# aslpavel/svgrasterize.py

Measured on AMD Instinct MI355X. Metric: Mpixels/sec AA coverage+composite (path-pixels/s; whole step: flatten+binning+coverage+composite; planned replay -- a frame with new geometry: value_replan), higher is better.
Workload: dtype f64 arithmetic, f32 RGBA store; 1 GPU; synthetic 4096 random closed cubic paths @ 4096x4096 (SURVEY 8d generator, splitmix64 0x5F3759DF); edges=783607

## Files before the change

### svgrasterize.py_amd/csrc/svgr_hip.hip

```cpp
#include <hip/hip_runtime.h>

#include <algorithm>
#include <atomic>
#include <cstdarg>
#include <cstddef>
#include <cmath>
#include <cstdio>
#include <cstring>
#include <ctime>
#include <initializer_list>
#include <new>
#include <string>
#include <type_traits>
#include <vector>
#include <memory>
#include <unordered_map>
#include <utility>

#include "../../include/svgr.h"
#include "svgr_core.h"

using namespace svgr;

static std::atomic<unsigned long long> g_n_launches{0};
// ... 719 lines not shown
        if (i0 + PER <= n) {
            ((int4*)(seg_off + i0))[0] = make_int4(o[0], o[1], o[2], o[3]);
            ((int4*)(seg_off + i0))[1] = make_int4(o[4], o[5], o[6], o[7]);
        } else {
#pragma unroll
            for (int k = 0; k < PER; ++k)
                if (i0 + k < n) seg_off[i0 + k] = o[k];
        }
        __syncthreads();
        if (tid == 0) s_run = run0 + all;
        __syncthreads();
    }
    if (tid == 0) seg_off[n] = s_run;
}

struct PathBin {
    int b0, nb;
    int pb_off;
    int cell_off;
};
__host__ __device__ __forceinline__ void path_ctiles(int c0, int cols, int vc0, int& ct0, int& nct) {
    span_ctiles(c0, cols, vc0, TC, ct0, nct);
}
static_assert(sizeof(PathBin) == 16, "PathBin is one dwordx4");

constexpr int PB_THREADS = 256;
constexpr int PB_CELLS = 80;
constexpr int PB_BANDS = 16;
static_assert(PB_BANDS * TR <= PB_THREADS && PB_BANDS <= PB_CELLS, "k_path_build: one lane group per band of the slab");
struct Slab {
    int p, band0, nb, k0;
    int nk, e_begin, e_end, pb_off;
    int r0, c0, rows, cols;
    int b0, cell_off, pad[2];
};
static_assert(sizeof(Slab) == 64, "Slab is four dwordx4");
__host__ __device__ __forceinline__ void slab_shape(int nb, int nct, int& bands_per, int& col_runs) {
    if (nct <= PB_CELLS) {
        bands_per = PB_CELLS / nct < PB_BANDS ? PB_CELLS / nct : PB_BANDS;
        col_runs = 1;
    } else {
        bands_per = 1;
        col_runs = (nct + PB_CELLS - 1) / PB_CELLS;
    }
    (void)nb;
}

__global__ __launch_bounds__(64) void k_path_bbox(const unsigned long long* __restrict__ pkeys, int n_paths, int has_vp,
                                                  int vr0, int vc0, int vrows, int vcols, int* __restrict__ bbox,
                                                  PathBin* __restrict__ bins, BatchDev* __restrict__ bd, int stats,
                                                  const int* __restrict__ plist, Slab* __restrict__ slabs, int slab_cap, Owner own,
                                                  const int* __restrict__ path_seg0, const int* __restrict__ seg_off, int edge_cap,
                                                  const int* __restrict__ slab_at) {
    const int pi = blockIdx.x * blockDim.x + threadIdx.x, lane = threadIdx.x & 63;
    const int p = plist ? (pi < n_paths ? plist[pi] : 0x7fffffff) : pi;
    if (plist) n_paths = pi < n_paths ? 0x7fffffff : 0;
    int e_begin = 0, e_end = 0;
    if (slabs && p < n_paths) {
        e_begin = seg_off[path_seg0[p]]; e_end = seg_off[path_seg0[p + 1]];
    }
    const bool reuse = slab_at != nullptr;
    PathBin old_bin;
    old_bin.b0 = old_bin.nb = old_bin.pb_off = old_bin.cell_off = 0;
    int4 old_bb = make_int4(0, 0, 0, 0);
    if (reuse && p < n_paths) { old_bin = bins[p]; old_bb = ((const int4*)bbox)[p]; }
    int out[4] = {0, 0, 0, 0};
    int pb0 = 0, pnb = 0, pnct = 0;
    int st_n = 0;
    unsigned long long st_px = 0;
    unsigned st_minr = 0, st_minc = 0, st_maxr = 0, st_maxc = 0;
    PathBox pb = path_box(0ull, 0ull, 0ull, 0ull, has_vp, vr0, vc0, vrows, vcols, TR, TC);
    if (p < n_paths) {
        const unsigned long long* k = pkeys + 4 * (size_t)p;
        pb = path_box(k[0], k[1], k[2], k[3], has_vp, vr0, vc0, vrows, vcols, TR, TC);
        if (pb.refused) atomicOr(&bd->err, 16);
        out[0] = pb.r0; out[1] = pb.c0; out[2] = pb.rows; out[3] = pb.cols;
        pb0 = pb.b0; pnb = pb.nb; pnct = pb.nct;
        if (pb.rows > 0 && pb.cols > 0) {
            st_n = 1;
            st_px = (unsigned long long)((long long)pb.rows * pb.cols);
            st_minr = (unsigned)(UNION_BIAS - pb.r0);
            st_minc = (unsigned)(UNION_BIAS - pb.c0);
            st_maxr = (unsigned)(UNION_BIAS + (pb.r0 + pb.rows));
            st_maxc = (unsigned)(UNION_BIAS + (pb.c0 + pb.cols));
        }
    }
    if (reuse && p < n_paths && !path_box_is(pb, old_bb.x, old_bb.y, old_bb.z, old_bb.w, old_bin.nb)) {
        atomicOr(&bd->err, 32);
        out[0] = old_bb.x; out[1] = old_bb.y; out[2] = old_bb.z; out[3] = old_bb.w;
        pb0 = old_bin.b0; pnb = old_bin.nb; pnct = 0;
        if (pnb > 0 && out[2] > 0 && out[3] > 0) {
            int ct0_;
// ... 42 lines not shown
        st_n += __shfl_xor(st_n, d);
        st_px += __shfl_xor(st_px, d);
        unsigned a = __shfl_xor(st_minr, d), b = __shfl_xor(st_minc, d), c = __shfl_xor(st_maxr, d), e = __shfl_xor(st_maxc, d);
        st_minr = a > st_minr ? a : st_minr; st_minc = b > st_minc ? b : st_minc;
        st_maxr = c > st_maxr ? c : st_maxr; st_maxc = e > st_maxc ? e : st_maxc;
    }
    if (stats && lane == 0 && st_n > 0) {
        atomicAdd(&bd->n_nonempty, st_n);
        atomicAdd(&bd->path_pixels, st_px);
        atomicMax(&bd->umin_r, st_minr);
        atomicMax(&bd->umin_c, st_minc);
        atomicMax(&bd->umax_r, st_maxr);
        atomicMax(&bd->umax_c, st_maxc);
    }
    const bool coop = slabs != nullptr && own.world <= 1;
    if (coop) {
        const bool fits = n_slabs > 0 && slab0 + n_slabs <= slab_cap;
        int t_sl;
        const int e_sl = wave_excl_scan(fits ? n_slabs : 0, lane, t_sl);
        const int eb = e_begin < edge_cap ? e_begin : edge_cap, ee = e_end < edge_cap ? e_end : edge_cap;
        for (int base = 0; base < t_sl; base += 64) {
            const int i = base + lane;
            int owner = 0;
#pragma unroll
            for (int step = 32; step >= 1; step >>= 1) {
                const int cand = owner + step;
                const int first = __shfl(e_sl, cand & 63);
                if (cand < 64 && first <= i) owner = cand;
            }
            const int o_first = __shfl(e_sl, owner), o_slab0 = __shfl(slab0, owner), o_p = __shfl(p, owner);
            const int o_pb0 = __shfl(pb0, owner), o_pnb = __shfl(pnb, owner), o_pnct = __shfl(pnct, owner);
            const int o_bper = __shfl(bands_per, owner), o_cruns = __shfl(col_runs, owner);
            const int o_eb = __shfl(eb, owner), o_ee = __shfl(ee, owner), o_off = __shfl(off, owner), o_cell = __shfl(cell_off, owner);
            const int o_r0 = __shfl(out[0], owner), o_c0 = __shfl(out[1], owner), o_rows = __shfl(out[2], owner), o_cols = __shfl(out[3], owner);
            if (i < t_sl) {
                const int j = i - o_first;
                const int br = o_cruns == 1 ? j : j / o_cruns, c = o_cruns == 1 ? 0 : j - br * o_cruns;
                const int bb = br * o_bper, be = bb + o_bper < o_pnb ? bb + o_bper : o_pnb;
                Slab sl;
                sl.p = o_p; sl.band0 = o_pb0 + bb; sl.nb = be - bb;
                sl.k0 = c * PB_CELLS; sl.nk = o_pnct - sl.k0 < PB_CELLS ? o_pnct - sl.k0 : PB_CELLS;
                sl.e_begin = o_eb; sl.e_end = o_ee; sl.pb_off = o_off;
                sl.r0 = o_r0; sl.c0 = o_c0; sl.rows = o_rows; sl.cols = o_cols;
                sl.b0 = o_pb0; sl.cell_off = o_cell;
                sl.pad[0] = sl.pad[1] = 0;
                slabs[o_slab0 + j] = sl;
            }
        }
    }
    if (slabs && n_slabs > 0 && !(coop && slab0 + n_slabs <= slab_cap)) {
        if (slab0 + n_slabs > slab_cap) {
            atomicOr(&bd->err, 4);
            for (int at = slab0; at < slab_cap; ++at) {
                Slab sl;
                memset(&sl, 0, sizeof sl);
                slabs[at] = sl;
            }
        } else {
            int at = slab0;
            e_begin = e_begin < edge_cap ? e_begin : edge_cap;
            e_end = e_end < edge_cap ? e_end : edge_cap;
            for (int bb = 0; bb < pnb; bb += bands_per) {
                const int be = bb + bands_per < pnb ? bb + bands_per : pnb;
                if (!owns_any(own, pb0 + bb, pb0 + be - 1)) continue;
                for (int c = 0; c < col_runs; ++c) {
                    Slab sl;
                    sl.p = p; sl.band0 = pb0 + bb; sl.nb = be - bb;
                    sl.k0 = c * PB_CELLS; sl.nk = pnct - sl.k0 < PB_CELLS ? pnct - sl.k0 : PB_CELLS;
                    sl.e_begin = e_begin; sl.e_end = e_end; sl.pb_off = off;
                    sl.r0 = out[0]; sl.c0 = out[1]; sl.rows = out[2]; sl.cols = out[3];
                    sl.b0 = pb0; sl.cell_off = cell_off;
                    sl.pad[0] = sl.pad[1] = 0;
                    slabs[at++] = sl;
                }
            }
        }
    }
    if (p < n_paths) {
        ((int4*)bbox)[p] = make_int4(out[0], out[1], out[2], out[3]);
        PathBin pbin;
        pbin.b0 = pb0; pbin.nb = pnb; pbin.pb_off = off; pbin.cell_off = cell_off;
        bins[p] = pbin;
    }
}

__device__ __forceinline__ bool edge_prepare(const double* __restrict__ edges, const int* __restrict__ edge_path,
                                             const int* __restrict__ bbox, int e, EdgeSetup& es, int& p, int& r0) {
    p = edge_path[e];
    const int4 bb = ((const int4*)bbox)[p];
    r0 = bb.x;
    const int rows = bb.z, cols = bb.w;
    if (rows <= 0 || cols <= 0) return false;
    const double o_r = (double)bb.x, o_c = (double)bb.y;
    const double* ed = edges + 4 * (size_t)e;
    double ar = ed[0] - o_r, ac = ed[1] - o_c, br = ed[2] - o_r, bc = ed[3] - o_c;
    es = edge_setup(ar, ac, br, bc, rows);
    if (!es.valid) return false;
    double cmin = ac < bc ? ac : bc;
    if (cmin >= (double)cols + 2.0) return false;
    return true;
}

__device__ __forceinline__ void band_rows(const EdgeSetup& es, int band, int vr0, int r0, int& ya, int& yb) {
    const int b0row = band * TR + vr0 - r0;
    ya = es.y_begin > b0row ? es.y_begin : b0row;
// ... 186 lines not shown

__device__ __forceinline__ int lds_col(int tcol) {
    static_assert((PX & (PX - 1)) == 0, "PX is a power of two");
    return tcol + (int)((unsigned)tcol / PX) * (CHUNK_STRIDE - PX);
}
__device__ __forceinline__ int lds_index(int trow, int tcol) {
    return __mul24(trow, ROW_STRIDE) + lds_col(tcol);
}
__device__ __forceinline__ int run_pieces(int tcol, int len) {
    return ((tcol + len - 1) / PX) - (tcol / PX) + 1;
}
__device__ __forceinline__ unsigned add_where(int trow, int tcol, int len) {
    return (unsigned)(lds_index(trow, tcol) * 8) | ((unsigned)(len - 1) << 16) | ((unsigned)(tcol & (PX - 1)) << 22);
}

struct EdgeLds {
    double p0y, p1y, dxdy, x;
};
__device__ __forceinline__ double replay_rows(double x, int y, int n, double p0y, double p1y, double dxdy) {
    if (n <= 0) return x;
    RowState st;
    st.x_next = x; st.x = x; st.d = 0.0;
    row_step(st, y, p0y, p1y, dxdy, 1.0);
    double xn = st.x_next;
    for (int k = 1; k < n; ++k) xn = xn + dxdy;
    return xn;
}
static_assert(sizeof(EdgeLds) == 32, "EdgeLds is two 16-byte LDS reads (its first row and direction ride in an int array beside it)");
constexpr int PB_BATCH = 256;
constexpr int PB_EPL = (PB_BATCH + PB_THREADS - 1) / PB_THREADS;
static_assert(PB_BATCH % 64 == 0 && PB_BATCH / 16 <= 32, "two-level search: at most 32 coarse entries, read four at a time");
static_assert(PB_BANDS * TR * PB_BATCH < (1 << 20) && PB_BATCH < (1 << 11), "stage() scans row counts and live flags in one packed word");
constexpr int PB_WAVES = 6;
__device__ __forceinline__ void pb_barrier() { asm volatile("s_waitcnt lgkmcnt(0)\n\ts_barrier" ::: "memory"); }
template <int MODE>
__global__ __launch_bounds__(PB_THREADS, PB_WAVES) void k_path_build(const Slab* __restrict__ slabs, const double* __restrict__ edges,
                                                           const int* __restrict__ pair_idx, const double* __restrict__ path_paint,
                                                           const uint8_t* __restrict__ path_rule, const int* __restrict__ path_group,
                                                           const int* __restrict__ path_grad, int vr0, int vc0, int n_ct, int mask_words,
                                                           unsigned long long* __restrict__ tile_mask, CellHdr* __restrict__ cell_hdr,
                                                           int cell_cap, const AddShards ash, TileAdd* __restrict__ adds,
                                                           int2* __restrict__ cell_plan, BatchDev* __restrict__ bd, Owner own, int stats, int det,
                                                           unsigned long long* __restrict__ dbg,
                                                           const unsigned long long* __restrict__ guard_keys, const int* __restrict__ guard_bbox,
                                                           const PathBin* __restrict__ guard_bins, int n_paths, int vrows, int vcols) {
#ifdef SVGR_DBG_PB_STAMP
#define PB_STAMP(i) do { if (threadIdx.x == 0 && dbg && blockIdx.x < 8192) dbg[8 * blockIdx.x + (i)] = __builtin_amdgcn_s_memrealtime(); } while (0)
#else
#define PB_STAMP(i) do { } while (0)
#endif
    constexpr bool PLANNED = MODE != 0;
    constexpr bool BOUNDED = MODE == 2;
    PB_STAMP(0);
    __shared__ __attribute__((aligned(16))) double s_sum[PB_CELLS * TR];
    __shared__ double s_left[TR];
    __shared__ int s_cnt[PB_CELLS], s_pos[PB_CELLS], s_plan_n[PB_CELLS];
    __shared__ unsigned s_rowb[PB_CELLS + 1];
    __shared__ __attribute__((aligned(16))) EdgeLds s_edge[PB_BATCH];
    __shared__ int s_eya[PB_BATCH];
    __shared__ __attribute__((aligned(16))) int s_pref[PB_BATCH + 4];
    __shared__ unsigned short s_start[PB_THREADS];
    __shared__ int s_wtot[PB_EPL][PB_THREADS / 64];
    __shared__ __attribute__((aligned(8))) int2 s_info[PB_CELLS];
    __shared__ unsigned s_rowm[PB_CELLS];
    __shared__ int s_ptot[PB_BANDS], s_pidx[PB_BANDS], s_base, s_ok;
    const int tid = threadIdx.x, lane = tid & 63, wave = tid >> 6;
    for (int i = tid; i < PB_CELLS * TR / 2; i += PB_THREADS) ((double2*)s_sum)[i] = make_double2(0.0, 0.0);
    for (int i = tid; i < PB_CELLS; i += PB_THREADS) {
        s_cnt[i] = 0; s_pos[i] = (int)0x80000000; s_plan_n[i] = 0; s_rowb[i] = 0u; s_info[i] = make_int2(0, 0);
    }
    if (tid < TR) s_left[tid] = 0.0;
    if (tid == 0) s_rowb[PB_CELLS] = 0u;
    const Slab sl = slabs[blockIdx.x];
    const bool guarding = MODE == 1 && guard_keys != nullptr;
    const int n_slabs_now = guarding ? (int)gridDim.x : bd->slab_cursor;
    if ((int)blockIdx.x >= n_slabs_now) return;
    if (sl.nb <= 0 || sl.nk <= 0) return;
    PB_STAMP(7);
    const int p = sl.p;
    const int r0 = sl.r0, c0 = sl.c0, rows = sl.rows, cols = sl.cols;
    int ct0, nct;
    path_ctiles(c0, cols, vc0, ct0, nct);
    const int x_first = vc0 + ct0 * TC - c0;
    const int e_begin = sl.e_begin, e_end = sl.e_end;
    const int sr0 = vr0 + sl.band0 * TR - r0, sr1 = sr0 + sl.nb * TR;
    const int n_cell = sl.nb * sl.nk;
    const double o_r = (double)r0, o_c = (double)c0;
    const int rl = path_rule[p], rule = rl & 1;
    const int group = path_group ? path_group[p] : -1;
    const int grad1 = path_grad ? path_grad[p] + 1 : 0;
    const double4 paint = ((const double4*)path_paint)[p];
    auto cell_of = [&](int g, int k) { return sl.cell_off + (sl.band0 + g - sl.b0) * nct + sl.k0 + k; };
    int s_per = 0;
    int2 my_plan = make_int2((int)0x80000000, 0);
    bool plan_pending = false;
    int my_pidx = 0;
    if ((tid & (TR - 1)) == 0 && tid / TR < sl.nb && owns_band(own, sl.band0 + tid / TR)) my_pidx = pair_idx[sl.pb_off + sl.band0 + tid / TR - sl.b0];
    if (PLANNED && !BOUNDED) {
        if (tid < n_cell) {
            const int g = tid / sl.nk, k = tid - g * sl.nk;
            const int cell = cell_of(g, k);
            if (cell < cell_cap) my_plan = cell_plan[cell];
        }
        plan_pending = true;
    }

    auto stage = [&](int eb, bool bounds = false) -> int {
        int cnt[PB_EPL], eya[PB_EPL];
        EdgeLds el[PB_EPL];
#pragma unroll
        for (int j = 0; j < PB_EPL; ++j) {
            const int e = eb + tid + j * PB_THREADS;
            cnt[j] = 0;
            el[j].p0y = el[j].p1y = el[j].dxdy = el[j].x = 0.0; eya[j] = 0;
            if (e < e_end && tid + j * PB_THREADS < PB_BATCH) {
                const double4 ed = ((const double4*)edges)[e];
                const double ar = ed.x - o_r, ac = ed.y - o_c, br = ed.z - o_r, bc = ed.w - o_c;
                const EdgeSetup es = edge_setup(ar, ac, br, bc, rows);
                const double cmin = ac < bc ? ac : bc;
                if (es.valid && !(cmin >= (double)cols + 2.0)) {
                    const int ya = es.y_begin > sr0 ? es.y_begin : sr0, yb = es.y_end < sr1 ? es.y_end : sr1;
                    if (ya < yb) {
                        cnt[j] = yb - ya;
                        el[j].p0y = es.p0y; el[j].p1y = es.p1y; el[j].dxdy = es.dxdy; el[j].x = replay_rows(es.x, es.y_begin, ya - es.y_begin, es.p0y, es.p1y, es.dxdy);
                        eya[j] = ya | (es.dir < 0.0 ? (int)0x80000000 : 0);
                    }
                }
            }
        }
#ifdef SVGR_DBG_PB_STAMP
        if (PLANNED && eb == e_begin) { asm volatile("s_waitcnt vmcnt(0)" ::: "memory"); PB_STAMP(5); }
#endif
        int excl[PB_EPL], wtot[PB_EPL];
#pragma unroll
        for (int j = 0; j < PB_EPL; ++j) excl[j] = wave_excl_scan(cnt[j] | ((cnt[j] > 0 ? 1 : 0) << 20), lane, wtot[j]);
        pb_barrier();
        if (PLANNED && plan_pending) {
            if (tid < PB_CELLS) { s_pos[tid] = my_plan.x; s_plan_n[tid] = my_plan.y; }
            plan_pending = false;
        }
        if (BOUNDED && bounds) {
#pragma unroll
            for (int j = 0; j < PB_EPL; ++j) {
                if (cnt[j] <= 0) continue;
                const int ya = eya[j] & 0x7fffffff, yb = ya + cnt[j];
                const double dx = el[j].dxdy;
                const double ylo = (double)ya > el[j].p0y ? (double)ya : el[j].p0y;
                for (int y0 = ya; y0 < yb;) {
                    const int vrow = r0 + y0 - vr0, band = vrow / TR;
// ... 154 lines not shown
            if (ne == 0) continue;
            const int ci = bl * sl.nk + (k - sl.k0);
            const int pos = __hip_atomic_fetch_add(&s_cnt[ci], ne, __ATOMIC_RELAXED, __HIP_MEMORY_SCOPE_WORKGROUP);
            __hip_atomic_fetch_add(&s_sum[ci * TR + trow], part, __ATOMIC_RELAXED, __HIP_MEMORY_SCOPE_WORKGROUP);
            __hip_atomic_fetch_or(&s_rowb[ci], 1u << trow, __ATOMIC_RELAXED, __HIP_MEMORY_SCOPE_WORKGROUP);
            if (STORE) {
                const int first = s_pos[ci];
                if (first < 0 || pos + ne > s_plan_n[ci]) continue;
                store_pieces(ra, trow, ca, cb, cell_c0, adds + ((size_t)first + pos));
            }
        }
    };
    auto emit_row = [&](const RowAt& ra) {
        if (!((ra.where >> 16) & 1)) return;
        const int bl = ra.where & 0xff, trow = (ra.where >> 8) & 0xff;
        int kf, kl;
        row_tiles(ra, kf, kl);
        kf = kf > sl.k0 ? kf : sl.k0;
        for (int k = kf; k <= kl; ++k) {
            int ca, cb;
            tile_cols(k, ca, cb);
            int ne = 0;
            const int cell_c0 = k * TC + x_first;
            record_adds(ra.x0i, ra.n, ra.v, ca, cb, [&](int, double) { ++ne; },
                        [&](int c, int len, double) { ne += run_pieces(c - cell_c0, len); });
            if (ne == 0) continue;
            const int ci = bl * sl.nk + (k - sl.k0);
            const int pos = __hip_atomic_fetch_add(&s_pos[ci], ne, __ATOMIC_RELAXED, __HIP_MEMORY_SCOPE_WORKGROUP);
            if (pos < 0) continue;
            store_pieces(ra, trow, ca, cb, cell_c0, adds + pos);
        }
    };

    const bool one_batch = e_end - e_begin <= PB_BATCH;
    int total = 0, n_rows = 0;
    if (BOUNDED) {
        for (int eb = e_begin; eb < e_end; eb += PB_BATCH) {
            total = stage(eb, true);
            n_rows += total;
        }
        PB_STAMP(1);
        static_assert(PB_CELLS <= 128, "the cells' places: a prefix sum by the first two waves");
        int room = 0, excl = 0;
        if (tid < 128) {
            const int bnd = tid < n_cell ? s_plan_n[tid] : 0;
            const int gg = tid < n_cell ? tid / sl.nk : 0, kk = tid < n_cell ? tid - gg * sl.nk : 0;
            const bool ends_here = cols - ((sl.k0 + kk) * TC + x_first) < TC;
            const int b_lo = vr0 + (sl.band0 + gg) * TR - r0;
            const int rin = (b_lo + TR < rows ? b_lo + TR : rows) - (b_lo > 0 ? b_lo : 0);
            room = bnd > 0 ? bnd + rin + (ends_here ? rin : 0) : 0;
            int wt;
            excl = wave_excl_scan(room, lane, wt);
            if (lane == 0) s_ptot[wave] = wt;
        }
        pb_barrier();
        if (tid == 0) {
            const int all = s_ptot[0] + s_ptot[1];
            const int sh = p % ash.n;
            int at = 0;
            if (all > 0) at = atomicAdd(&bd->shard[sh].add_cursor, all);
            int ok = 1;
            if ((long long)at + all > (long long)ash.cap[sh]) { atomicOr(&bd->err, 64); ok = 0; }
            s_base = ash.base[sh] + at;
            s_ok = ok;
        }
        pb_barrier();
        if (tid < n_cell) s_pos[tid] = room > 0 && s_ok ? s_base + (wave ? s_ptot[0] : 0) + excl : (int)0x80000000;
        pb_barrier();
        if (one_batch) {
            for_rows(total, [&](const RowAt& ra) { count_row(ra, std::true_type{}); });
        } else {
            for (int eb = e_begin; eb < e_end; eb += PB_BATCH) {
                const int tot = stage(eb);
                for_rows(tot, [&](const RowAt& ra) { count_row(ra, std::true_type{}); });
            }
        }
    } else
    for (int eb = e_begin; eb < e_end; eb += PB_BATCH) {
        total = stage(eb);
        PB_STAMP(1);
        n_rows += total;
        if (PLANNED) for_rows(total, [&](const RowAt& ra) { count_row(ra, std::true_type{}); });
        else for_rows(total, [&](const RowAt& ra) { count_row(ra, std::false_type{}); });
    }
    if (stats && tid == 0 && n_rows > 0) atomicAdd(&bd->bseg_cursor, n_rows);
    if (guarding && __builtin_amdgcn_readfirstlane(wave) == 0) {
        const int grid = (int)gridDim.x, g0 = ((int)blockIdx.x + grid - grid / 2) % grid;
        for (int g = g0; g * 64 < n_paths; g += grid) {
            const int q = g * 64 + lane;
            if (q >= n_paths) continue;
            const unsigned long long* k = guard_keys + 4 * (size_t)q;
            const int4 bb = ((const int4*)guard_bbox)[q];
            const PathBox pb = path_box(k[0], k[1], k[2], k[3], 1, vr0, vc0, vrows, vcols, TR, TC);
            if (pb.refused) atomicOr(&bd->err, 16);
            if (!path_box_is(pb, bb.x, bb.y, bb.z, bb.w, guard_bins[q].nb)) atomicOr(&bd->err, 32);
        }
    }
    pb_barrier();
    PB_STAMP(2);
    auto write_cell = [&](int g, int k, int cls, double cin, unsigned cm, unsigned sm, int own_n, int n_list, int add0, int row_l, int idx,
                          bool slab_ok) -> bool {
        const int band = sl.band0 + g;
        const int cell = cell_of(g, k);
        const bool mask_ok = (unsigned)(idx >> 6) < (unsigned)mask_words;
        if (!(cell < cell_cap && slab_ok && mask_ok) || (PLANNED && cls == 2 && add0 < 0)) {
            if (row_l == 0) atomicOr(&bd->err, 32);
            return false;
        }
        CellHdr* hd = cell_hdr + cell;
        if (cls == 1) hd->carry[row_l] = cin;
        const int cell_c0 = (sl.k0 + k) * TC + x_first;
        const unsigned below = (1u << row_l) - 1u;
        const int n_carry = __popc(cm);
        if (((cm >> row_l) & 1u) && adds) {
            store_add(adds + ((size_t)add0 + own_n + __popc(cm & below)), add_where(row_l, cell_c0 < 0 ? -cell_c0 : 0, 1), cin);
        }
        if (((sm >> row_l) & 1u) && adds) {
            store_add(adds + ((size_t)add0 + own_n + n_carry + __popc(sm & below)), add_where(row_l, cols - cell_c0, 1), __builtin_nan(""));
        }
        if (row_l == 0) {
            unsigned long long* const mw = tile_mask + ((size_t)band * n_ct + ct0 + sl.k0 + k) * 2 * mask_words + (idx >> 6);
            const unsigned long long mbit = 1ull << (idx & 63);
            atomicOr(mw, mbit);
            if (cls == 2) atomicOr(mw + mask_words, mbit);
            hd->paint[0] = paint.x; hd->paint[1] = paint.y; hd->paint[2] = paint.z; hd->paint[3] = paint.w;
            hd->r0 = r0; hd->c0 = c0; hd->rows = rows; hd->cols = cols;
            hd->bits = rule | (((rl >> 1) & 3) << 1) | (cls << 3) | (grad1 << 5);
            hd->n_add = n_list; hd->add0 = add0; hd->p = p;
            hd->group = group;
        }
        return true;
    };
// ... 2438 lines not shown
        SVGR_LAUNCH(k_path_rows, grid1((size_t)ns), dim3(256), 0, st, (const double*)b->segs.p, (const uint8_t*)b->seg_kind.p,
                           (const int*)b->seg_path.p, (const double*)b->path_m6.p, ns, b->prow());
        prow = b->prow();
    }
    const int n_bands_vp = use_vp ? (b->vp[2] + TR - 1) / TR : 0;
    if (upto <= 1) {
        if (upto == 1) {
            if (int rc = b->seg_cnt.ensure((size_t)ns + 1)) return rc;
            if (int rc = b->seg_off.ensure((size_t)ns + 2)) return rc;
            if (int rc = b->lane_off.ensure(((size_t)ns << fl_sub) + 1)) return rc;
            if (listed || prow) HIPCHK(hipMemsetAsync(b->seg_cnt.p, 0, sizeof(int) * ((size_t)ns + 1), st));
        }
        if (ns > 0) {
            auto launch_cnt = [&](auto kern) {
                SVGR_LAUNCH(kern, fgrid, dim3(FL_BLOCK), 0, st, (const double*)b->segs.p,
                                   (const uint8_t*)b->seg_kind.p, (const int*)b->seg_path.p, (const double*)b->path_m6.p, ns,
                                   b->thr, (double*)nullptr, (int*)nullptr, b->shards, b->pkeys(), b->bd(), b->own, b->vp[0],
                                   n_bands_vp, prow, seg_list, n_items, upto == 1 ? b->seg_cnt.p : (int*)nullptr, (const int*)nullptr,
                                   use_vp ? b->vp[3] : 0 ,
                                   upto == 1 ? b->lane_off.p : (int*)nullptr, (int*)nullptr, (unsigned long long*)nullptr);
            };
            if (fl_sub == 6) launch_cnt(k_flatten<false, false, 6>); else launch_cnt(k_flatten<false, false, 5>);
        }
        if (upto == 1 && !b->late_scan)
            SVGR_LAUNCH(k_seg_scan, dim3(1), dim3(1024), 0, st, (const int*)b->seg_cnt.p, ns, b->seg_off.p);
        if (upto == 0 || (upto == 1 && b->census_bbox)) {
            b->slabs_current = false;
            SVGR_LAUNCH(k_path_bbox, grid1((size_t)std::max(np_walk, 1), 64), dim3(64), 0, st, (const unsigned long long*)b->pkeys(),
                               np_walk, use_vp ? 1 : 0, b->vp[0], b->vp[1], b->vp[2], b->vp[3], b->bbox.p, b->bins.p, b->bd(), 1, plist,
                               (Slab*)nullptr, 0, b->own, (const int*)nullptr, (const int*)nullptr, 0, (const int*)nullptr);
        }
        return 0;
    }
    if (ns > 0) {
        const bool lane_places = !b->safe_path;
        auto launch_fl = [&](auto kern, int* places) {
            SVGR_LAUNCH(kern, fgrid, dim3(FL_BLOCK), 0, st, (const double*)b->segs.p,
                               (const uint8_t*)b->seg_kind.p, (const int*)b->seg_path.p, (const double*)b->path_m6.p, ns, b->thr,
                               b->edges.p, b->edge_path.p, b->shards, b->pkeys(), b->bd(), b->own, b->vp[0],
                               n_bands_vp, prow, seg_list, n_items, (int*)nullptr, (const int*)b->seg_off.p,
                               cap_i32(std::min(b->edge_path.cap, b->edges.cap / 4)), places, (int*)nullptr, (unsigned long long*)nullptr);
        };
        const bool placed_fl = lane_places && b->lane_off.p && b->lane_off.cap >= ((size_t)ns << fl_sub);
        if (b->fl_scan) {
            auto launch_scan = [&](auto kern) {
                SVGR_LAUNCH(kern, fgrid, dim3(FL_BLOCK), 0, st, (const double*)b->segs.p,
                                   (const uint8_t*)b->seg_kind.p, (const int*)b->seg_path.p, (const double*)b->path_m6.p, ns, b->thr,
                                   b->edges.p, b->edge_path.p, b->shards, b->pkeys(), b->bd(), b->own, b->vp[0],
                                   n_bands_vp, prow, seg_list, n_items, b->seg_cnt.p, (const int*)nullptr,
                                   cap_i32(std::min(b->edge_path.cap, b->edges.cap / 4)), b->lane_off.p, b->seg_off.p, b->scan_state());
            };
            if (fl_sub == 6) launch_scan(k_flatten<true, false, 6, true>); else launch_scan(k_flatten<true, false, 5, true>);
        } else if (fl_sub == 6) {
            if (placed_fl) launch_fl(k_flatten<true, true, 6>, b->lane_off.p); else launch_fl(k_flatten<true, false, 6>, (int*)nullptr);
        } else {
            if (placed_fl) launch_fl(k_flatten<true, true, 5>, b->lane_off.p); else launch_fl(k_flatten<true, false, 5>, (int*)nullptr);
        }
    }
    const bool keep_lists = upto >= 4 && b->planned && b->slab_at_valid && use_vp && !b->safe_path;
    const bool placed = b->planned && b->add_places && b->slab_at_valid && !b->count_adds_only && b->cell_plan.p != nullptr;
    const svgr_batch::SlabsMade slabs_now{b->slabs.p, b->bbox.p, b->bins.p, b->slab_at.p, b->n_slabs, b->n_paths, {b->vp[0], b->vp[1], b->vp[2], b->vp[3]}};
    const bool slabs_for_plan = keep_lists && b->own.world <= 1 && !listed && ns > 0 && b->n_slabs > 0 && b->n_slabs <= (int64_t)cap_i32(b->slabs.cap);
    const bool keep_slabs = slabs_for_plan && placed && b->slabs_current && b->slabs_made == slabs_now;
    if (!keep_slabs) {
        SVGR_LAUNCH(k_path_bbox, grid1((size_t)std::max(np_walk, 1), 64), dim3(64), 0, st, (const unsigned long long*)b->pkeys(), np_walk,
                           use_vp ? 1 : 0, b->vp[0], b->vp[1], b->vp[2], b->vp[3], b->bbox.p, b->bins.p, b->bd(), b->planned ? 0 : 1, plist,
                           upto >= 3 ? b->slabs.p : (Slab*)nullptr, (int)std::min<int64_t>(cap_i32(b->slabs.cap), b->n_slabs) , b->own,
                           (const int*)b->path_seg0.p, (const int*)b->seg_off.p,
                           cap_i32(std::min(b->edge_path.cap, b->edges.cap / 4)),
                           upto >= 4 && b->planned && b->slab_at_valid ? (const int*)b->slab_at.p : (const int*)nullptr);
        b->slabs_current = slabs_for_plan && !b->slab_order_late;
        b->slab_order_late = false;
        b->slabs_made = slabs_now;
    }
    if (upto == 2) return 0;
    const int owned = count_owned_bands(b->own, b->n_bands);
    const bool clear_in_be = owned > 0 && !keep_lists && upto >= 4 && !b->masks_zeroed && b->tile_mask.p && b->own.world <= 1;
    if (owned > 0 && !keep_lists)
        SVGR_LAUNCH(k_band_entries, dim3(owned), dim3(BE_BLOCK), 0, st, (const PathBin*)b->bins.p, np_walk, plist,
                           (const int*)b->bbox.p, b->band_start.p, b->band_count.p, b->band_item0.p, b->entries.p,
                           b->pair_idx.p, cap_i32(std::min(b->entries.cap, b->pair_idx.cap)),
                           upto >= 4 ? cap_i32(b->items.cap) : 0x7fffffff, b->vp[1], b->bd(), b->own,
                           upto >= 4 && b->planned && use_vp && !b->safe_path ? 1 : 0,
                           clear_in_be ? b->tile_mask.p : (unsigned long long*)nullptr, b->n_ctiles() * 2 * b->mask_words);
    if (clear_in_be) b->masks_zeroed = true;
    if (upto == 3) return 0;
    if (!b->masks_zeroed && b->tile_mask.p) {
        HIPCHK(hipMemsetAsync(b->tile_mask.p, 0, b->mask_bytes(), st));
        b->masks_zeroed = true;
    }
    unsigned long long* pb_dbg = nullptr;
#ifdef SVGR_DBG_PB_STAMP
    {
        static unsigned long long* buf = nullptr;
        if (!buf) { (void)hipMalloc((void**)&buf, 8 * 8 * 8192); (void)hipMemset(buf, 0, 8 * 8 * 8192); }
        pb_dbg = buf;
    }
#endif
    if (b->n_slabs > 0) {
        b->masks_zeroed = false;
        auto launch_pb = [&](auto kern) {
            SVGR_LAUNCH(kern, dim3((unsigned)b->n_slabs), dim3(PB_THREADS), 0, st, (const Slab*)b->slabs.p, (const double*)b->edges.p,
                               (const int*)b->pair_idx.p, (const double*)b->path_paint.p, (const uint8_t*)b->path_rule.p,
                               b->n_groups > 0 ? (const int*)b->path_group.p : (const int*)nullptr,
                               b->n_grads > 0 ? (const int*)b->path_grad.p : (const int*)nullptr, b->vp[0], b->vp[1], b->n_ctiles(), b->mask_words,
                               b->tile_mask.p, b->cell_hdr.p, cap_i32(std::min(b->cell_hdr.cap, b->cell_plan.cap)), b->add_shards,
                               b->count_adds_only ? (TileAdd*)nullptr : b->adds.p, b->cell_plan.p, b->bd(), b->own, b->planned ? 0 : 1,
                               b->deterministic ? 1 : 0, pb_dbg, keep_slabs ? (const unsigned long long*)b->pkeys() : (const unsigned long long*)nullptr,
                               (const int*)b->bbox.p, (const PathBin*)b->bins.p, np, b->vp[2], b->vp[3]);
        };
        const bool bounded = !placed && !b->count_adds_only && b->adds.p && b->adds_roomy && !b->safe_path && !getenv("SVGR_SAFE_PATH");
        if (placed) launch_pb(k_path_build<1>); else if (bounded) launch_pb(k_path_build<2>); else launch_pb(k_path_build<0>);
#ifdef SVGR_DBG_PB_STAMP
        if (pb_dbg && b->planned && !b->count_adds_only) {
            static int n_dump = 0;
            if (++n_dump == 20) {
                HIPCHK(hipStreamSynchronize(st));
                const size_t n = (size_t)std::min<int64_t>(b->n_slabs, 8192);
                std::vector<unsigned long long> h(8 * n);
                HIPCHK(hipMemcpy(h.data(), pb_dbg, sizeof(unsigned long long) * h.size(), hipMemcpyDeviceToHost));
                double ph[5] = {0, 0, 0, 0, 0}, rows_ = 0;
                unsigned long long lo = ~0ull, hi = 0;
                for (size_t i = 0; i < n; ++i) {
                    for (int q = 0; q < 5; ++q) ph[q] += (double)(h[8 * i + q + 1] - h[8 * i + q]);
                    rows_ += (double)h[8 * i + 6];
                    lo = std::min(lo, h[8 * i]); hi = std::max(hi, h[8 * i + 3]);
                }
                double s_rec = 0, s_edges = 0;
                for (size_t i = 0; i < n; ++i) { s_rec += (double)(h[8 * i + 7] - h[8 * i]); s_edges += (double)(h[8 * i + 5] - h[8 * i + 7]); }
                fprintf(stderr, "[pb stamp] %zu slabs, mean us: stage %.2f (slab record %.2f, edges landed +%.2f)  passA %.2f  walk %.2f | rows/slab %.0f | span %.1f us\n", n,
                        ph[0] / n / 100, s_rec / n / 100, s_edges / n / 100, ph[1] / n / 100, ph[2] / n / 100, rows_ / n, (double)(hi - lo) / 100);
                if (const char* f = getenv("SVGR_DBG_PB_DUMP")) { if (FILE* fp = fopen(f, "wb")) { fwrite(h.data(), 8, h.size(), fp); fclose(fp); } }
            }
        }
#endif
    }
    if (owned > 0 && b->n_ctiles() > 0) {
        SVGR_LAUNCH(k_tile_lists, dim3(owned), dim3(TL_BLOCK), 0, st, (const int*)b->band_start.p, (const int*)b->band_item0.p,
                           (const TileEntry*)b->entries.p, b->tile_mask.p, b->mask_words, b->n_ctiles(), b->vp[1], b->own, owned,
                           b->tile_info.p, b->pages.p, b->items.p, (const CellHdr*)b->cell_hdr.p, cap_i32(b->items.cap), cap_i32(b->cell_hdr.cap), b->bd(),
                           keep_lists ? (const PathBin*)b->bins.p : (const PathBin*)nullptr, (const int*)b->bbox.p);
        b->masks_zeroed = true;
    }
    return 0;
}
// ... 2330 lines not shown
```

Before: 810,100 Mpixels/s.

## Fuse planned curve flattening into path-build slabs, skipping the global edge buffer

On planned replay with reusable slabs, the separate flatten kernel is skipped. Each path-build slab re-flattens its path's segments batch by batch straight into shared memory, using the precomputed lane placements, so edges are never written to or read from global memory. The bbox guard check is now folded from keys computed during this flatten, and a small new kernel covers paths that have no slabs. The costs are repeated flattening for paths split across many slabs, an extra barrier per batch, and lower occupancy (5 waves instead of 6).

Measured after the change: 688,900 Mpixels/s. 15.0% lower.

```diff
diff --git a/svgrasterize.py_amd/csrc/svgr_hip.hip b/svgrasterize.py_amd/csrc/svgr_hip.hip
--- a/svgrasterize.py_amd/csrc/svgr_hip.hip
+++ b/svgrasterize.py_amd/csrc/svgr_hip.hip
@@ -775,7 +775,8 @@
     int p, band0, nb, k0;
     int nk, e_begin, e_end, pb_off;
     int r0, c0, rows, cols;
-    int b0, cell_off, pad[2];
+    int b0, cell_off;
+    int seg0, n_seg;
 };
 static_assert(sizeof(Slab) == 64, "Slab is four dwordx4");
 __host__ __device__ __forceinline__ void slab_shape(int nb, int nct, int& bands_per, int& col_runs) {
@@ -798,9 +799,10 @@
     const int pi = blockIdx.x * blockDim.x + threadIdx.x, lane = threadIdx.x & 63;
     const int p = plist ? (pi < n_paths ? plist[pi] : 0x7fffffff) : pi;
     if (plist) n_paths = pi < n_paths ? 0x7fffffff : 0;
-    int e_begin = 0, e_end = 0;
+    int e_begin = 0, e_end = 0, seg_first = 0, seg_n = 0;
     if (slabs && p < n_paths) {
-        e_begin = seg_off[path_seg0[p]]; e_end = seg_off[path_seg0[p + 1]];
+        seg_first = path_seg0[p]; seg_n = path_seg0[p + 1] - seg_first;
+        e_begin = seg_off[seg_first]; e_end = seg_off[seg_first + seg_n];
     }
     const bool reuse = slab_at != nullptr;
     PathBin old_bin;
@@ -909,6 +911,7 @@
             const int o_pb0 = __shfl(pb0, owner), o_pnb = __shfl(pnb, owner), o_pnct = __shfl(pnct, owner);
             const int o_bper = __shfl(bands_per, owner), o_cruns = __shfl(col_runs, owner);
             const int o_eb = __shfl(eb, owner), o_ee = __shfl(ee, owner), o_off = __shfl(off, owner), o_cell = __shfl(cell_off, owner);
+            const int o_seg = __shfl(seg_first, owner), o_nseg = __shfl(seg_n, owner);
             const int o_r0 = __shfl(out[0], owner), o_c0 = __shfl(out[1], owner), o_rows = __shfl(out[2], owner), o_cols = __shfl(out[3], owner);
             if (i < t_sl) {
                 const int j = i - o_first;
@@ -920,7 +923,7 @@
                 sl.e_begin = o_eb; sl.e_end = o_ee; sl.pb_off = o_off;
                 sl.r0 = o_r0; sl.c0 = o_c0; sl.rows = o_rows; sl.cols = o_cols;
                 sl.b0 = o_pb0; sl.cell_off = o_cell;
-                sl.pad[0] = sl.pad[1] = 0;
+                sl.seg0 = o_seg; sl.n_seg = o_nseg;
                 slabs[o_slab0 + j] = sl;
             }
         }
@@ -947,7 +950,7 @@
                     sl.e_begin = e_begin; sl.e_end = e_end; sl.pb_off = off;
                     sl.r0 = out[0]; sl.c0 = out[1]; sl.rows = out[2]; sl.cols = out[3];
                     sl.b0 = pb0; sl.cell_off = cell_off;
-                    sl.pad[0] = sl.pad[1] = 0;
+                    sl.seg0 = seg_first; sl.n_seg = seg_n;
                     slabs[at++] = sl;
                 }
             }
@@ -1200,9 +1203,132 @@
 static_assert(PB_BATCH % 64 == 0 && PB_BATCH / 16 <= 32, "two-level search: at most 32 coarse entries, read four at a time");
 static_assert(PB_BANDS * TR * PB_BATCH < (1 << 20) && PB_BATCH < (1 << 11), "stage() scans row counts and live flags in one packed word");
 constexpr int PB_WAVES = 6;
+constexpr int PB_WAVES_FUSED = 5;
 __device__ __forceinline__ void pb_barrier() { asm volatile("s_waitcnt lgkmcnt(0)\n\ts_barrier" ::: "memory"); }
-template <int MODE>
-__global__ __launch_bounds__(PB_THREADS, PB_WAVES) void k_path_build(const Slab* __restrict__ slabs, const double* __restrict__ edges,
+struct FlattenSrc {
+    const double* segs;
+    const uint8_t* kind;
+    const double* path_m6;
+    const int* seg_off;
+    const int* lane_off;
+    const int* path_seg0;
+    double thr;
+    int sub;
+    int n_bands;
+};
+struct FlKeys {
+    unsigned long long k[4];
+};
+template <class Store>
+__device__ __forceinline__ void flatten_planned_lane(const FlattenSrc& fl, int seg, int sub, int p, Owner own, int vr0,
+                                                     BatchDev* __restrict__ bd, FlKeys& keys, Store&& store) {
+    const int segl = 1 << fl.sub;
+    const int so0 = fl.seg_off[seg], so1 = fl.seg_off[seg + 1];
+    const int first = fl.lane_off[(size_t)seg * segl + sub];
+    const int nxt = sub == segl - 1 ? so1 - so0 : fl.lane_off[(size_t)seg * segl + sub + 1];
+    const int n_plan = nxt - first, base_p = so0 + first;
+    double node[8];
+    int mode = 0;
+    const double* m6 = fl.path_m6 + 6 * (size_t)p;
+    if (fl.kind[seg] == SVGR_SEG_LINE) {
+        if (sub == 0) {
+            double c[4];
+            load_seg_points(fl.segs, seg, m6, 2, c);
+            node[0] = c[0]; node[1] = c[1]; node[6] = c[2]; node[7] = c[3];
+            mode = 1;
+        }
+    } else {
+        load_seg_points(fl.segs, seg, m6, 4, node);
+        mode = 2;
+        for (int l = 0; l < fl.sub; ++l) {
+            if (cubic_flatness(node) < fl.thr) {
+                mode = (sub & ((1 << (fl.sub - l)) - 1)) == 0 ? 1 : 0;
+                break;
+            }
+            if ((sub >> (fl.sub - 1 - l)) & 1) cubic_right_inplace(node); else cubic_left_inplace(node);
+        }
+    }
+    bool keep = true;
+    if (fl.n_bands > 0 && mode != 0) {
+        double rlo = node[0] < node[6] ? node[0] : node[6], rhi = node[0] < node[6] ? node[6] : node[0];
+        if (mode == 2) {
+            rlo = fmin(rlo, fmin(node[2], node[4]));
+            rhi = fmax(rhi, fmax(node[2], node[4]));
+        }
+        const double v_lo = (double)vr0 - 4.0, v_hi = (double)vr0 + (double)fl.n_bands * TR + 4.0;
+        rlo = rlo < v_lo ? v_lo : (rlo > v_hi ? v_hi : rlo);
+        rhi = rhi < v_lo ? v_lo : (rhi > v_hi ? v_hi : rhi);
+        int ba = (clamp_to_int(floor(rlo)) - 1 - vr0) / TR, bb = (clamp_to_int(ceil(rhi)) + 1 - vr0) / TR;
+        ba = clamp_to_int(floor(rlo)) - 1 - vr0 < 0 ? 0 : ba;
+        bb = bb > fl.n_bands - 1 ? fl.n_bands - 1 : bb;
+        keep = ba <= bb && owns_any(own, ba, bb);
+    }
+    double mnr = INFINITY, mnc = INFINITY, mxr = -INFINITY, mxc = -INFINITY;
+    auto track = [&](double r, double c) {
+        mnr = r < mnr ? r : mnr; mxr = r > mxr ? r : mxr;
+        mnc = c < mnc ? c : mnc; mxc = c > mxc ? c : mxc;
+    };
+    int n_found = 0;
+    bool ovf = false;
+    if (mode == 1) {
+        track(node[0], node[1]);
+        track(node[6], node[7]);
+        n_found = 1;
+        if (n_plan >= 1) store(base_p, node[0], node[1], node[6], node[7]);
+    } else if (mode == 2) {
+        track(node[0], node[1]);
+        int at = 0;
+        n_found = flatten_subtree<1>(node, fl.thr, kMaxFlattenDepth - fl.sub, [&](double r0_, double c0_, double r1, double c1) {
+            track(r1, c1);
+            if (at < n_plan) store(base_p + at, r0_, c0_, r1, c1);
+            ++at;
+        }, ovf);
+    }
+    if (ovf) atomicOr(&bd->err, 1);
+    if (keep && n_found != n_plan) atomicOr(&bd->err, 2);
+    if (mnr <= mxr) {
+        const unsigned long long a = ~f64_key(mnr), b = ~f64_key(mnc), c = f64_key(mxr), d = f64_key(mxc);
+        keys.k[0] = a > keys.k[0] ? a : keys.k[0]; keys.k[1] = b > keys.k[1] ? b : keys.k[1];
+        keys.k[2] = c > keys.k[2] ? c : keys.k[2]; keys.k[3] = d > keys.k[3] ? d : keys.k[3];
+    }
+}
+__device__ __forceinline__ void fl_keys_fold_wave(FlKeys& keys) {
+#pragma unroll
+    for (int d = 1; d < 64; d <<= 1)
+#pragma unroll
+        for (int i = 0; i < 4; ++i) {
+            const unsigned long long o = __shfl_xor(keys.k[i], d);
+            keys.k[i] = o > keys.k[i] ? o : keys.k[i];
+        }
+}
+
+__global__ __launch_bounds__(64) void k_guard_slabless(const PathBin* __restrict__ bins, const int* __restrict__ bbox, int n_paths,
+                                                       int vr0, int vc0, int vrows, int vcols, Owner own, BatchDev* __restrict__ bd,
+                                                       const FlattenSrc fl) {
+    const int lane = threadIdx.x, q = (int)blockIdx.x * 64 + lane;
+    const bool mine = q < n_paths && bins[q].nb <= 0;
+    FlKeys qk;
+    qk.k[0] = qk.k[1] = qk.k[2] = qk.k[3] = 0ull;
+    for (unsigned long long m = __ballot(mine); m; m &= m - 1ull) {
+        const int src = __ffsll((long long)m) - 1, qq = (int)blockIdx.x * 64 + src;
+        const int qs0 = fl.path_seg0[qq], qs1 = fl.path_seg0[qq + 1];
+        FlKeys wk;
+        wk.k[0] = wk.k[1] = wk.k[2] = wk.k[3] = 0ull;
+        for (int L = lane; qs0 + (L >> fl.sub) < qs1; L += 64)
+            flatten_planned_lane(fl, qs0 + (L >> fl.sub), L & ((1 << fl.sub) - 1), qq, own, vr0, bd, wk,
+                                 [](int, double, double, double, double) {});
+        fl_keys_fold_wave(wk);
+        if (lane == src) qk = wk;
+    }
+    if (!mine) return;
+    const int4 bb = ((const int4*)bbox)[q];
+    const PathBox pb = path_box(qk.k[0], qk.k[1], qk.k[2], qk.k[3], 1, vr0, vc0, vrows, vcols, TR, TC);
+    if (pb.refused) atomicOr(&bd->err, 16);
+    if (!path_box_is(pb, bb.x, bb.y, bb.z, bb.w, bins[q].nb)) atomicOr(&bd->err, 32);
+}
+
+template <int MODE, bool FUSED = false>
+__global__ __launch_bounds__(PB_THREADS, FUSED ? PB_WAVES_FUSED : PB_WAVES) void k_path_build(const Slab* __restrict__ slabs, const double* __restrict__ edges,
                                                            const int* __restrict__ pair_idx, const double* __restrict__ path_paint,
                                                            const uint8_t* __restrict__ path_rule, const int* __restrict__ path_group,
                                                            const int* __restrict__ path_grad, int vr0, int vc0, int n_ct, int mask_words,
@@ -1211,7 +1337,10 @@
                                                            int2* __restrict__ cell_plan, BatchDev* __restrict__ bd, Owner own, int stats, int det,
                                                            unsigned long long* __restrict__ dbg,
                                                            const unsigned long long* __restrict__ guard_keys, const int* __restrict__ guard_bbox,
-                                                           const PathBin* __restrict__ guard_bins, int n_paths, int vrows, int vcols) {
+                                                           const PathBin* __restrict__ guard_bins, int n_paths, int vrows, int vcols,
+                                                           const FlattenSrc fl) {
+    static_assert(!FUSED || MODE == 1, "the fused flatten takes the plan's places");
+    static_assert(!FUSED || (PB_EPL == 1 && sizeof(double4) == sizeof(EdgeLds)), "the flattened batch lies in s_edge, slot = thread");
 #ifdef SVGR_DBG_PB_STAMP
 #define PB_STAMP(i) do { if (threadIdx.x == 0 && dbg && blockIdx.x < 8192) dbg[8 * blockIdx.x + (i)] = __builtin_amdgcn_s_memrealtime(); } while (0)
 #else
@@ -1232,6 +1361,7 @@
     __shared__ __attribute__((aligned(8))) int2 s_info[PB_CELLS];
     __shared__ unsigned s_rowm[PB_CELLS];
     __shared__ int s_ptot[PB_BANDS], s_pidx[PB_BANDS], s_base, s_ok;
+    __shared__ unsigned long long s_keys[FUSED ? PB_THREADS / 64 : 1][4];
     const int tid = threadIdx.x, lane = tid & 63, wave = tid >> 6;
     for (int i = tid; i < PB_CELLS * TR / 2; i += PB_THREADS) ((double2*)s_sum)[i] = make_double2(0.0, 0.0);
     for (int i = tid; i < PB_CELLS; i += PB_THREADS) {
@@ -1240,7 +1370,7 @@
     if (tid < TR) s_left[tid] = 0.0;
     if (tid == 0) s_rowb[PB_CELLS] = 0u;
     const Slab sl = slabs[blockIdx.x];
-    const bool guarding = MODE == 1 && guard_keys != nullptr;
+    const bool guarding = MODE == 1 && (FUSED || guard_keys != nullptr);
     const int n_slabs_now = guarding ? (int)gridDim.x : bd->slab_cursor;
     if ((int)blockIdx.x >= n_slabs_now) return;
     if (sl.nb <= 0 || sl.nk <= 0) return;
@@ -1282,7 +1412,7 @@
             cnt[j] = 0;
             el[j].p0y = el[j].p1y = el[j].dxdy = el[j].x = 0.0; eya[j] = 0;
             if (e < e_end && tid + j * PB_THREADS < PB_BATCH) {
-                const double4 ed = ((const double4*)edges)[e];
+                const double4 ed = FUSED ? ((const double4*)s_edge)[tid + j * PB_THREADS] : ((const double4*)edges)[e];
                 const double ar = ed.x - o_r, ac = ed.y - o_c, br = ed.z - o_r, bc = ed.w - o_c;
                 const EdgeSetup es = edge_setup(ar, ac, br, bc, rows);
                 const double cmin = ac < bc ? ac : bc;
@@ -1503,6 +1633,38 @@
         }
     };
 
+    FlKeys keys;
+    keys.k[0] = keys.k[1] = keys.k[2] = keys.k[3] = 0ull;
+    const int seg0 = sl.seg0, seg1 = seg0 + sl.n_seg;
+    int seg_lo = seg0;
+    auto flatten_batch = [&](int eb, int eb_end, bool last) {
+        if (eb > e_begin) {
+            for (;;) {
+                const int s = seg_lo + 1 + lane;
+                const int n = __popcll(__ballot(s <= seg1 && fl.seg_off[s < seg1 ? s : seg1] < eb));
+                seg_lo += n;
+                if (n < 64) break;
+            }
+            seg_lo = seg_lo < seg1 ? seg_lo : seg1;
+        }
+        double4* const raw = (double4*)s_edge;
+        const int segl = 1 << fl.sub;
+        for (int L = tid;; L += PB_THREADS) {
+            const int seg = seg_lo + (L >> fl.sub), sub = L & (segl - 1);
+            if (seg >= seg1) break;
+            const int so0 = fl.seg_off[seg];
+            if (so0 >= eb_end && !last) break;
+            const int first = fl.lane_off[(size_t)seg * segl + sub];
+            const int nxt = sub == segl - 1 ? fl.seg_off[seg + 1] - so0 : fl.lane_off[(size_t)seg * segl + sub + 1];
+            const int at0 = so0 + first, at1 = so0 + nxt;
+            const bool starts_here = at0 >= eb && (at0 < eb_end || last);
+            if (!(starts_here || (at0 < eb && at1 > eb))) continue;
+            flatten_planned_lane(fl, seg, sub, p, own, vr0, bd, keys, [&](int e, double r0_, double c0_, double r1_, double c1_) {
+                if (e >= eb && e < eb_end) raw[e - eb] = make_double4(r0_, c0_, r1_, c1_);
+            });
+        }
+    };
+
     const bool one_batch = e_end - e_begin <= PB_BATCH;
     int total = 0, n_rows = 0;
     if (BOUNDED) {
@@ -1547,7 +1709,13 @@
             }
         }
     } else
-    for (int eb = e_begin; eb < e_end; eb += PB_BATCH) {
+    for (int eb = e_begin; eb < e_end || (FUSED && eb == e_begin); eb += PB_BATCH) {
+        if (FUSED) {
+            const int eb_end = eb + PB_BATCH < e_end ? eb + PB_BATCH : e_end;
+            if (eb > e_begin) pb_barrier();
+            flatten_batch(eb, eb_end, eb_end >= e_end);
+            pb_barrier();
+        }
         total = stage(eb);
         PB_STAMP(1);
         n_rows += total;
@@ -1555,7 +1723,11 @@
         else for_rows(total, [&](const RowAt& ra) { count_row(ra, std::false_type{}); });
     }
     if (stats && tid == 0 && n_rows > 0) atomicAdd(&bd->bseg_cursor, n_rows);
-    if (guarding && __builtin_amdgcn_readfirstlane(wave) == 0) {
+    if (FUSED) {
+        fl_keys_fold_wave(keys);
+        if (lane == 0) { s_keys[wave][0] = keys.k[0]; s_keys[wave][1] = keys.k[1]; s_keys[wave][2] = keys.k[2]; s_keys[wave][3] = keys.k[3]; }
+    }
+    if (!FUSED && guarding && __builtin_amdgcn_readfirstlane(wave) == 0) {
         const int grid = (int)gridDim.x, g0 = ((int)blockIdx.x + grid - grid / 2) % grid;
         for (int g = g0; g * 64 < n_paths; g += grid) {
             const int q = g * 64 + lane;
@@ -1569,6 +1741,16 @@
     }
     pb_barrier();
     PB_STAMP(2);
+    if (FUSED && tid == 0) {
+        unsigned long long k[4];
+        for (int i = 0; i < 4; ++i) {
+            k[i] = s_keys[0][i];
+            for (int w = 1; w < PB_THREADS / 64; ++w) k[i] = s_keys[w][i] > k[i] ? s_keys[w][i] : k[i];
+        }
+        const PathBox pb = path_box(k[0], k[1], k[2], k[3], 1, vr0, vc0, vrows, vcols, TR, TC);
+        if (pb.refused) atomicOr(&bd->err, 16);
+        if (!path_box_is(pb, r0, c0, rows, cols, guard_bins[p].nb)) atomicOr(&bd->err, 32);
+    }
     auto write_cell = [&](int g, int k, int cls, double cin, unsigned cm, unsigned sm, int own_n, int n_list, int add0, int row_l, int idx,
                           bool slab_ok) -> bool {
         const int band = sl.band0 + g;
@@ -4073,7 +4255,14 @@
         }
         return 0;
     }
-    if (ns > 0) {
+    const bool keep_lists = upto >= 4 && b->planned && b->slab_at_valid && use_vp && !b->safe_path;
+    const bool placed = b->planned && b->add_places && b->slab_at_valid && !b->count_adds_only && b->cell_plan.p != nullptr;
+    const svgr_batch::SlabsMade slabs_now{b->slabs.p, b->bbox.p, b->bins.p, b->slab_at.p, b->n_slabs, b->n_paths, {b->vp[0], b->vp[1], b->vp[2], b->vp[3]}};
+    const bool slabs_for_plan = keep_lists && b->own.world <= 1 && !listed && ns > 0 && b->n_slabs > 0 && b->n_slabs <= (int64_t)cap_i32(b->slabs.cap);
+    const bool keep_slabs = slabs_for_plan && placed && b->slabs_current && b->slabs_made == slabs_now;
+    const bool lane_places_ok = !b->safe_path && b->lane_off.p && b->lane_off.cap >= ((size_t)ns << fl_sub) && b->seg_off.p;
+    const bool fused = keep_slabs && lane_places_ok && !b->fl_scan && !prow;
+    if (ns > 0 && !fused) {
         const bool lane_places = !b->safe_path;
         auto launch_fl = [&](auto kern, int* places) {
             SVGR_LAUNCH(kern, fgrid, dim3(FL_BLOCK), 0, st, (const double*)b->segs.p,
@@ -4098,11 +4287,6 @@
             if (placed_fl) launch_fl(k_flatten<true, true, 5>, b->lane_off.p); else launch_fl(k_flatten<true, false, 5>, (int*)nullptr);
         }
     }
-    const bool keep_lists = upto >= 4 && b->planned && b->slab_at_valid && use_vp && !b->safe_path;
-    const bool placed = b->planned && b->add_places && b->slab_at_valid && !b->count_adds_only && b->cell_plan.p != nullptr;
-    const svgr_batch::SlabsMade slabs_now{b->slabs.p, b->bbox.p, b->bins.p, b->slab_at.p, b->n_slabs, b->n_paths, {b->vp[0], b->vp[1], b->vp[2], b->vp[3]}};
-    const bool slabs_for_plan = keep_lists && b->own.world <= 1 && !listed && ns > 0 && b->n_slabs > 0 && b->n_slabs <= (int64_t)cap_i32(b->slabs.cap);
-    const bool keep_slabs = slabs_for_plan && placed && b->slabs_current && b->slabs_made == slabs_now;
     if (!keep_slabs) {
         SVGR_LAUNCH(k_path_bbox, grid1((size_t)std::max(np_walk, 1), 64), dim3(64), 0, st, (const unsigned long long*)b->pkeys(), np_walk,
                            use_vp ? 1 : 0, b->vp[0], b->vp[1], b->vp[2], b->vp[3], b->bbox.p, b->bins.p, b->bd(), b->planned ? 0 : 1, plist,
@@ -4148,10 +4332,17 @@
                                b->tile_mask.p, b->cell_hdr.p, cap_i32(std::min(b->cell_hdr.cap, b->cell_plan.cap)), b->add_shards,
                                b->count_adds_only ? (TileAdd*)nullptr : b->adds.p, b->cell_plan.p, b->bd(), b->own, b->planned ? 0 : 1,
                                b->deterministic ? 1 : 0, pb_dbg, keep_slabs ? (const unsigned long long*)b->pkeys() : (const unsigned long long*)nullptr,
-                               (const int*)b->bbox.p, (const PathBin*)b->bins.p, np, b->vp[2], b->vp[3]);
+                               (const int*)b->bbox.p, (const PathBin*)b->bins.p, np, b->vp[2], b->vp[3],
+                               FlattenSrc{(const double*)b->segs.p, (const uint8_t*)b->seg_kind.p, (const double*)b->path_m6.p, (const int*)b->seg_off.p,
+                                          (const int*)b->lane_off.p, (const int*)b->path_seg0.p, b->thr, fl_sub, n_bands_vp});
         };
         const bool bounded = !placed && !b->count_adds_only && b->adds.p && b->adds_roomy && !b->safe_path && !getenv("SVGR_SAFE_PATH");
-        if (placed) launch_pb(k_path_build<1>); else if (bounded) launch_pb(k_path_build<2>); else launch_pb(k_path_build<0>);
+        if (fused)
+            SVGR_LAUNCH(k_guard_slabless, grid1((size_t)np, 64), dim3(64), 0, st, (const PathBin*)b->bins.p, (const int*)b->bbox.p, np, b->vp[0], b->vp[1],
+                        b->vp[2], b->vp[3], b->own, b->bd(),
+                        FlattenSrc{(const double*)b->segs.p, (const uint8_t*)b->seg_kind.p, (const double*)b->path_m6.p, (const int*)b->seg_off.p,
+                                   (const int*)b->lane_off.p, (const int*)b->path_seg0.p, b->thr, fl_sub, n_bands_vp});
+        if (fused) launch_pb(k_path_build<1, true>); else if (placed) launch_pb(k_path_build<1>); else if (bounded) launch_pb(k_path_build<2>); else launch_pb(k_path_build<0>);
 #ifdef SVGR_DBG_PB_STAMP
         if (pb_dbg && b->planned && !b->count_adds_only) {
             static int n_dump = 0;
```
